# mfalxa/fakepta

Measured on AMD Instinct MI355X. Metric: residual samples/sec (TOA×realization) for 100-psr HD GWB; % FP64 peak, higher is better.
Workload: dtype f64

## Files before the change

fakepta_amd/csrc/fused_sched.h:

```cpp
#pragma once
#include <cstdint>

#if defined(__HIPCC__)
#define FPTA_SCHED_HD __host__ __device__
#else
#define FPTA_SCHED_HD
#endif

namespace fpta {

constexpr int kFusedShapeAny = 0;
constexpr int kFusedShapeGenLoad = 1;
constexpr int kFusedShapeLoad = 2;
constexpr int kFusedSlotAny = -1, kFusedSlotNone = 0, kFusedSlotGen = 1, kFusedSlotLoad = 2;
FPTA_SCHED_HD constexpr int fused_shape_nsig(int shape) {
  return shape == kFusedShapeGenLoad ? 2 : shape == kFusedShapeLoad ? 1 : 0;
}
FPTA_SCHED_HD constexpr int fused_shape_slot(int shape, int s, int i) {
  return shape == kFusedShapeAny       ? kFusedSlotAny
         : shape == kFusedShapeGenLoad ? (i == 0 ? kFusedSlotGen : (s == 0 && i == 1 ? kFusedSlotLoad : kFusedSlotNone))
                                       : (s == 0 && i == 0 ? kFusedSlotLoad : kFusedSlotNone);
}

FPTA_SCHED_HD constexpr int fused_shape_match(int n_sig, const int32_t* n_terms, const int32_t (*kind)[2]) {
  return n_sig == 2 && n_terms[0] == 2 && kind[0][0] == 0 && kind[0][1] == 1 && n_terms[1] == 1 && kind[1][0] == 0
             ? kFusedShapeGenLoad
         : n_sig == 1 && n_terms[0] == 1 && kind[0][0] == 1 ? kFusedShapeLoad
                                                            : kFusedShapeAny;
}

FPTA_SCHED_HD constexpr int32_t fused_ksteps(int32_t nm, int par) { return (((nm + (par ? 0 : 1)) >> 1) + 3) >> 2; }
FPTA_SCHED_HD constexpr int32_t fused_groups(int32_t nm) { return (fused_ksteps(nm, 0) + 1) >> 1; }

FPTA_SCHED_HD constexpr int32_t fused_iterations(int32_t ng0, int32_t ng1) { return ng0 > ng1 ? ng0 : ng1; }
FPTA_SCHED_HD constexpr bool fused_steps(int32_t jng, int32_t g) { return g < jng; }
FPTA_SCHED_HD constexpr bool fused_draw_loads(int32_t ng_s, int32_t g, bool last) { return last || g + 1 < ng_s; }
FPTA_SCHED_HD constexpr bool fused_draws(int32_t ng_s, int32_t g, bool last, bool nx) { return last ? nx : g + 1 < ng_s; }
FPTA_SCHED_HD constexpr int32_t fused_draw_group(int32_t g, bool last) { return last ? 0 : g + 1; }

}

#undef FPTA_SCHED_HD
```

fakepta_amd/csrc/grid_fused.hip:

```cpp
#include <hip/hip_runtime.h>
#include <hip/hip_ext.h>
#include <algorithm>
#include <atomic>
#include <type_traits>

#include "fused_device.h"

namespace fpta {

#ifndef FPTA_FUSED_DFT_PRIO
#define FPTA_FUSED_DFT_PRIO 3
#endif
#ifndef FPTA_HALF_STORE16
#define FPTA_HALF_STORE16 0
#endif
#ifndef FPTA_HALF_AHEAD
#define FPTA_HALF_AHEAD 2
#endif
constexpr int kFusedHalfAhead = FPTA_HALF_AHEAD;
#ifndef FPTA_HALF_PIN
#define FPTA_HALF_PIN 0
#endif

#ifndef FPTA_FUSED_CUT
#define FPTA_FUSED_CUT 0
#endif

namespace {

template <int NS>
struct FusedOps {
  int c;
  i32x4 ci;
  dbl2 b[NS];
  int row[NS];
};
template <int NS>
struct FusedOpsH {
  int c;
  i32x4 ci;
  dbl2 b[2][NS / 2];
  int row[2][NS];
};

__device__ __forceinline__ uint32_t dpp_u32_xor1(uint32_t x) {
  return (uint32_t)__builtin_amdgcn_update_dpp(0, (int)x, 0xB1, 0xF, 0xF, false);
}
__device__ __forceinline__ void bm_half(uint32_t wl, uint32_t wa, double& zc, double& zs) {
  double sn, cs;
  const double r = bm_sqrt(-2.0 * bm_log_u32(wl));
  bm_sincos2pi_u32(wa, sn, cs);
  zc = r * cs;
  zs = r * sn;
}
__device__ __forceinline__ void fused_mix_tile(const FusedMix& m, int k, int rg, int pg, int lane) {
  constexpr int NT = kFusedMixGroup / 16;
  const int lr = lane & 15, lg = lane >> 4;
  const int r = 16 * rg + lr;
  const bool rv = r < m.n_real;
  const uint64_t g = (uint64_t)(m.real0 + r);
  const int p0 = kFusedMixGroup * pg;
  int qe[NT];
  int qmax = 0;
#pragma unroll
  for (int t = 0; t < NT; ++t) {
    const int pt = p0 + 16 * t;
    qe[t] = pt < m.P ? min(m.lower ? min(m.P, pt + 16) : m.P, m.n_q) : 0;
    qmax = max(qmax, qe[t]);
  }
  d4 acc[NT][2];
#pragma unroll
  for (int t = 0; t < NT; ++t) acc[t][0] = acc[t][1] = d4{0.0, 0.0, 0.0, 0.0};
  const double* __restrict__ lt = m.LT + p0 + lr;
  const bool paired = (m.real0 & 1) == 0;
  const int e = lr & 1;
  const uint32_t ctr3 = (uint32_t)(g >> 1);
  for (int q0 = 0; q0 < qmax; q0 += 8) {
    double a0[NT], a1[NT];
#pragma unroll
    for (int t = 0; t < NT; ++t) {
      a0[t] = q0 < qe[t] ? ld_global(lt + (int64_t)(q0 + lg) * m.lt_ld + 16 * t) : 0.0;
      a1[t] = q0 + 4 < qe[t] ? ld_global(lt + (int64_t)(q0 + 4 + lg) * m.lt_ld + 16 * t) : 0.0;
    }
    double zc0, zs0, zc1, zs1;
    if (paired) {
      const u32x4 v = philox4x32_10({(uint32_t)k, (uint32_t)(q0 + 4 * e + lg), (uint32_t)m.seg, ctr3}, m.k0, m.k1);
      const uint32_t r0 = dpp_u32_xor1(e ? v.x : v.z), r1 = dpp_u32_xor1(e ? v.y : v.w);
      bm_half(e ? r0 : v.x, e ? r1 : v.y, zc0, zs0);
      bm_half(e ? v.z : r0, e ? v.w : r1, zc1, zs1);
    } else {
      gp_normal2((uint32_t)k, (uint32_t)(q0 + lg), (uint32_t)m.seg, g, m.k0, m.k1, zc0, zs0);
      gp_normal2((uint32_t)k, (uint32_t)(q0 + 4 + lg), (uint32_t)m.seg, g, m.k0, m.k1, zc1, zs1);
    }
    const bool ok0 = rv && q0 + lg < m.n_q, ok1 = rv && q0 + 4 + lg < m.n_q;
    zc0 = ok0 ? zc0 : 0.0;
    zs0 = ok0 ? zs0 : 0.0;
    zc1 = ok1 ? zc1 : 0.0;
    zs1 = ok1 ? zs1 : 0.0;
#pragma unroll
    for (int t = 0; t < NT; ++t)
      if (q0 < qe[t]) {
        acc[t][0] = __builtin_amdgcn_mfma_f64_16x16x4f64(a0[t], zc0, acc[t][0], 0, 0, 0);
        acc[t][1] = __builtin_amdgcn_mfma_f64_16x16x4f64(a0[t], zs0, acc[t][1], 0, 0, 0);
      }
#pragma unroll
    for (int t = 0; t < NT; ++t)
      if (q0 + 4 < qe[t]) {
        acc[t][0] = __builtin_amdgcn_mfma_f64_16x16x4f64(a1[t], zc1, acc[t][0], 0, 0, 0);
        acc[t][1] = __builtin_amdgcn_mfma_f64_16x16x4f64(a1[t], zs1, acc[t][1], 0, 0, 0);
      }
  }
  const double am = ld_global(m.amp + k);
#pragma unroll
  for (int t = 0; t < NT; ++t)
#pragma unroll
    for (int h = 0; h < 2; ++h)
#pragma unroll
      for (int gg = 0; gg < 4; ++gg) {
        const int p = p0 + 16 * t + lg + 4 * gg;
        if (p < m.P) m.coef[((int64_t)p * m.K + m.col0 + 2 * k + h) * m.R_pad + r] = am * acc[t][h][gg];
      }
}

}

template <int NQ, bool ODD, bool GEN, bool HALF, int SHAPE>
__device__ __forceinline__ void grid_fused_body(const SynthArgs& a, const GridBand& band, const FusedArgs& f,
                                                int32_t n_rb, int32_t n_items) {
  static_assert(kFusedTerms == 2 && kFusedMaxSig == 2, "fused_shape_slot's slots and signals (c0, c1)");
  static_assert(SHAPE == kFusedShapeAny || GEN == (SHAPE == kFusedShapeGenLoad), "a shape fixes whether terms are drawn");
  static_assert(kFusedReal == 32 && kFusedPitch == 32 && kFusedGroupModes * kFusedReal / 2 == 64 * kFusedDW,
                "two realization tiles; one (mode, realization pair) of a 16-mode group per DFT lane");
  static_assert(!HALF || (NQ % 4 == 0 && kGridTT == 2 * kFusedHalfTT), "half bands: whole row groups, two halves");
  extern __shared__ __attribute__((aligned(16))) double lds[];
  const FusedQueue queue(n_items, f.queue);
  const int wave = __builtin_amdgcn_readfirstlane(threadIdx.x >> 6);
  const int lane = threadIdx.x & 63;
  const int lr = lane & 15, lg = lane >> 4;
  double* __restrict__ ring = lds + f.ring_off;
  uint32_t* sync = (uint32_t*)(ring + 2 * kFusedMaxSig * kFusedSlot);
  volatile int* qitem = (volatile int*)(sync + 4);
  if (threadIdx.x == 0) {
    *sync = 0u;
    ((volatile int*)sync)[8] = 0;
    ((volatile int*)sync)[9] = 0;
    qitem[0] = queue.fetch();
    qitem[1] = qitem[0] >= 0 ? queue.fetch() : -1;
  }
  __syncthreads();
  auto item_of = [&](int k) { return __builtin_amdgcn_readfirstlane(qitem[k & 3]); };
  auto finish = [&]() {
    if (threadIdx.x == 0) {
      __threadfence();
      const uint32_t done = __hip_atomic_fetch_add(f.queue + 8, 1u, __ATOMIC_ACQ_REL, __HIP_MEMORY_SCOPE_AGENT);
      if (done == gridDim.x - 1)
        for (int i = 0; i < kFusedQueueWords; ++i)
          __hip_atomic_store(f.queue + i, 0u, __ATOMIC_RELAXED, __HIP_MEMORY_SCOPE_AGENT);
    }
  };
  auto mix_tiles = [&]() {
    if (f.mix.n_tiles <= 0) return;
    __builtin_amdgcn_s_setprio(0);
    const int n_pg = (f.mix.P + kFusedMixGroup - 1) / kFusedMixGroup, n_rg = f.mix.R_pad >> 4;
    for (;;) {
      int t = 0;
      if (lane == 0)
        t = (int)__hip_atomic_fetch_add(f.queue + kFusedMixWord, 1u, __ATOMIC_RELAXED, __HIP_MEMORY_SCOPE_AGENT);
      t = __builtin_amdgcn_readfirstlane(t);
      if (t >= f.mix.n_tiles) break;
      const int pg = t % n_pg, kr = t / n_pg;
      const int k = kr / n_rg;
      fused_mix_tile(f.mix, k, kr - k * n_rg, pg, lane);
    }
  };
  if (item_of(0) < 0) {
    finish();
    return;
  }

  volatile int* ccnt = (volatile int*)(sync + 8);
  struct Geo {
    int p, r0, c0, n;
    int64_t toa0;
    bool valid;
  };
  auto geo = [&](int k) {
    Geo g;
    const int item = item_of(k);
    g.valid = item >= 0;
    const int it = g.valid ? item : 0;
    g.p = it / n_rb;
    g.r0 = (it - g.p * n_rb) * kFusedReal;
    g.c0 = ld_uniform(f.psr_c0 + g.p);
    g.n = g.valid ? ld_uniform(f.psr_c0 + g.p + 1) - g.c0 : 0;
    g.toa0 = ld_uniform(a.offs + g.p);
    return g;
  };
  auto ticket = [&](int k) {
    int t = 0;
    if (lane == 0)
      t = __hip_atomic_fetch_add((int*)ccnt + (k & 1), 1, __ATOMIC_RELAXED, __HIP_MEMORY_SCOPE_WORKGROUP);
    return __builtin_amdgcn_readfirstlane(t);
  };
  auto lane_now = [&]() {
    int v = lane;
    asm volatile("" : "+v"(v));
    return v;
  };
  using Ops = typename std::conditional<HALF, FusedOpsH<NQ>, FusedOps<NQ>>::type;
  using OpsJ = typename std::conditional<HALF, FusedOpsH<NQ>, FusedOps<(NQ < 8 ? NQ : 8)>>::type;
  auto load_half = [&](int cc, auto& o, int ln) {
    {
      constexpr int NS = sizeof(o.row[0]) / sizeof(o.row[0][0]);
      o.c = cc;
      o.ci = *(const i32x4*)(f.h.chunks + cc);
      const int lgo = ln >> 4, lro = ln & 15;
#pragma unroll
      for (int h = 0; h < 2; ++h) {
        const i32x4* __restrict__ rt = (const i32x4*)(f.h.lrows + (((int64_t)cc * 2 + h) * 4 + lgo) * f.h.fq);
#pragma unroll
        for (int q4 = 0; q4 < NS / 4; ++q4) {
          const i32x4 r4 = rt[q4];
          o.row[h][4 * q4] = r4.x;
          o.row[h][4 * q4 + 1] = r4.y;
          o.row[h][4 * q4 + 2] = r4.z;
          o.row[h][4 * q4 + 3] = r4.w;
        }
        const double* __restrict__ wp =
            f.h.wd + ((int64_t)cc * 2 + h) * f.h.vmax * kFusedHalfTT + (lgo * kFusedHalfTT + lro) * 2;
#pragma unroll
        for (int qp = 0; qp < NS / 2; ++qp) o.b[h][qp] = *(const dbl2*)(wp + qp * 8 * kFusedHalfTT);
      }
    }
  };
  auto load_full = [&](int cc, auto& o, int ln) {
    constexpr int NS = sizeof(o.row) / sizeof(o.row[0]);
    o.c = cc;
    o.ci = *(const i32x4*)(band.chunks + cc);
    const int lgo = ln >> 4, lro = ln & 15;
    const i32x4* __restrict__ rt = (const i32x4*)(f.lrows + ((int64_t)cc * 4 + lgo) * f.fq);
    const double* __restrict__ wp = band.wd + ((int64_t)cc * band.vmax + lgo) * kGridTT + 2 * lro;
#pragma unroll
    for (int q4 = 0; q4 < NS / 4; ++q4) {
      const i32x4 r4 = rt[q4];
      o.row[4 * q4] = r4.x;
      o.row[4 * q4 + 1] = r4.y;
      o.row[4 * q4 + 2] = r4.z;
      o.row[4 * q4 + 3] = r4.w;
    }
#pragma unroll
    for (int q = 0; q < NS; ++q) o.b[q] = *(const dbl2*)(wp + 4 * kGridTT * q);
  };
  auto load = [&](int cc, auto& o, int ln) {
    if constexpr (HALF)
      load_half(cc, o, ln);
    else
      load_full(cc, o, ln);
  };
  auto process_half = [&](const Geo& g, const auto& cur, auto& pf, int ln) {
    constexpr int NS = sizeof(cur.row[0]) / sizeof(cur.row[0][0]);
    const int lg = ln >> 4, lr = ln & 15;
    const int lds_lane = 2 * lr;
    const int ty = __builtin_amdgcn_readfirstlane(cur.ci.y), tc = __builtin_amdgcn_readfirstlane(cur.ci.z);
    const int nqw = __builtin_amdgcn_readfirstlane(cur.ci.w);
    const int nq[2] = {nqw & 0xFFFF, nqw >> 16};
    FPTA_DCHECK(nq[0] > 0, "k_grid_fused half band steps", nq[0], 1 << 20);
    d4 acc[2][2];
#pragma unroll
    for (int h = 0; h < 2; ++h)
#pragma unroll
      for (int i = 0; i < 2; ++i) acc[h][i] = d4{0.0, 0.0, 0.0, 0.0};
    {
      constexpr int DA = kFusedHalfAhead;
      const int nqm = min(max(nq[0], nq[1]), NS);
      dbl2 an[2][NS];
      auto rd = [&](int q) {
#pragma unroll
        for (int h = 0; h < 2; ++h) an[h][q] = *(const dbl2*)(lds + cur.row[h][q] * kFusedPitch + lds_lane);
      };
#pragma unroll
      for (int q = 0; q < DA && q < NS; ++q) rd(q);
#pragma unroll
      for (int q = 0; q < NS; ++q) {
        if (q < nqm) {
          if (q + DA < NS) rd(q + DA);
          if (FPTA_HALF_PIN) __builtin_amdgcn_sched_barrier(0);
          const double b0 = (q & 1) ? cur.b[0][q >> 1].y : cur.b[0][q >> 1].x;
          const double b1 = (q & 1) ? cur.b[1][q >> 1].y : cur.b[1][q >> 1].x;
          acc[0][0] = __builtin_amdgcn_mfma_f64_16x16x4f64(an[0][q].x, b0, acc[0][0], 0, 0, 0);
          acc[0][1] = __builtin_amdgcn_mfma_f64_16x16x4f64(an[0][q].y, b0, acc[0][1], 0, 0, 0);
          acc[1][0] = __builtin_amdgcn_mfma_f64_16x16x4f64(an[1][q].x, b1, acc[1][0], 0, 0, 0);
          acc[1][1] = __builtin_amdgcn_mfma_f64_16x16x4f64(an[1][q].y, b1, acc[1][1], 0, 0, 0);
        }
      }
    }
    pf.lap(1);
#pragma unroll
    for (int h = 0; h < 2; ++h)
      for (int q = NS; q < nq[h]; ++q) {
        const int64_t hc = (int64_t)cur.c * 2 + h;
        const int row = f.h.lrows[(hc * 4 + lg) * f.h.fq + q];
        const double bv = f.h.wd[hc * f.h.vmax * kFusedHalfTT + fused_half_weight_index(4 * q + lg, lr)];
        const dbl2 av = *(const dbl2*)(lds + row * kFusedPitch + lds_lane);
        acc[h][0] = __builtin_amdgcn_mfma_f64_16x16x4f64(av.x, bv, acc[h][0], 0, 0, 0);
        acc[h][1] = __builtin_amdgcn_mfma_f64_16x16x4f64(av.y, bv, acc[h][1], 0, 0, 0);
      }
    pf.lap(4);
    __builtin_amdgcn_sched_barrier(0);
    const int64_t t0 = g.toa0 + ty;
    if ((FPTA_FUSED_CUT & 8) && acc[0][0][0] != -1.25e300) return;
    if (FPTA_HALF_STORE16 && tc == kGridTT && g.r0 + kFusedReal <= a.n_real && ((t0 | a.ldo) & 1) == 0 &&
        a.ldo < ((int64_t)1 << 26)) {
      const bool odd = lr & 1;
      const uint32_t vo = (uint32_t)(((int64_t)2 * lg * a.ldo + (odd ? 15 + lr : lr)) * 8);
      const char* base = (const char*)(a.out + t0 + (int64_t)g.r0 * a.ldo);
#pragma unroll
      for (int i = 0; i < 2; ++i)
#pragma unroll
        for (int gg = 0; gg < 4; ++gg) {
          const double send = odd ? acc[0][i][gg] : acc[1][i][gg];
          const double recv = dpp_xor1(send);
          const dbl2 v = odd ? dbl2{recv, acc[1][i][gg]} : dbl2{acc[0][i][gg], recv};
          __builtin_nontemporal_store(v, (dbl2*)((char*)base + (int64_t)(8 * gg + i) * a.ldo * 8 + vo));
        }
    } else if (tc == kGridTT && g.r0 + kFusedReal <= a.n_real && a.ldo < ((int64_t)1 << 26)) {
      const uint32_t vo = (uint32_t)(((int64_t)2 * lg * a.ldo + lr) * 8);
      const char* base = (const char*)(a.out + t0 + (int64_t)g.r0 * a.ldo);
#pragma unroll
      for (int h = 0; h < 2; ++h)
#pragma unroll
        for (int i = 0; i < 2; ++i)
#pragma unroll
          for (int gg = 0; gg < 4; ++gg)
            __builtin_nontemporal_store(acc[h][i][gg],
                                        (double*)((char*)base + ((int64_t)(8 * gg + i) * a.ldo + 16 * h) * 8 + vo));
    } else {
#pragma unroll
      for (int h = 0; h < 2; ++h) {
        if (16 * h + lr >= tc) continue;
#pragma unroll
        for (int i = 0; i < 2; ++i)
#pragma unroll
          for (int gg = 0; gg < 4; ++gg) {
            const int r = g.r0 + 2 * (lg + 4 * gg) + i;
            if (r < a.n_real) a.out[t0 + 16 * h + lr + (int64_t)r * a.ldo] = acc[h][i][gg];
          }
      }
    }
    pf.lap(2);
  };
  auto process_full = [&](const Geo& g, const auto& cur, auto& pf, int ln) {
    constexpr int NS = sizeof(cur.row) / sizeof(cur.row[0]);
    const int lg = ln >> 4, lr = ln & 15;
    const int lds_lane = 2 * lr;
    const int ty = __builtin_amdgcn_readfirstlane(cur.ci.y), tc = __builtin_amdgcn_readfirstlane(cur.ci.z);
    const int nq = __builtin_amdgcn_readfirstlane(cur.ci.w) >> 2;
    FPTA_DCHECK(nq > 0, "k_grid_fused band steps", nq, 1 << 20);
    d4 acc[2][2];
#pragma unroll
    for (int e = 0; e < 2; ++e)
#pragma unroll
      for (int i = 0; i < 2; ++i) acc[e][i] = d4{0.0, 0.0, 0.0, 0.0};
    {
      dbl2 an = *(const dbl2*)(lds + cur.row[0] * kFusedPitch + lds_lane);
#pragma unroll
      for (int q = 0; q < NS; ++q) {
        if (q < nq) {
          const dbl2 av = an;
          if (q + 1 < NS) an = *(const dbl2*)(lds + cur.row[q + 1] * kFusedPitch + lds_lane);
          const dbl2 bv = cur.b[q];
          acc[0][0] = __builtin_amdgcn_mfma_f64_16x16x4f64(av.x, bv.x, acc[0][0], 0, 0, 0);
          acc[0][1] = __builtin_amdgcn_mfma_f64_16x16x4f64(av.y, bv.x, acc[0][1], 0, 0, 0);
          acc[1][0] = __builtin_amdgcn_mfma_f64_16x16x4f64(av.x, bv.y, acc[1][0], 0, 0, 0);
          acc[1][1] = __builtin_amdgcn_mfma_f64_16x16x4f64(av.y, bv.y, acc[1][1], 0, 0, 0);
        }
      }
    }
    pf.lap(1);
    for (int q = NS; q < nq; ++q) {
      const int v = 4 * q + lg;
      const int row = f.lrows[((int64_t)cur.c * 4 + lg) * f.fq + q];
      const dbl2 bv = *(const dbl2*)(band.wd + ((int64_t)cur.c * band.vmax + v) * kGridTT + 2 * lr);
      const dbl2 av = *(const dbl2*)(lds + row * kFusedPitch + lds_lane);
      acc[0][0] = __builtin_amdgcn_mfma_f64_16x16x4f64(av.x, bv.x, acc[0][0], 0, 0, 0);
      acc[0][1] = __builtin_amdgcn_mfma_f64_16x16x4f64(av.y, bv.x, acc[0][1], 0, 0, 0);
      acc[1][0] = __builtin_amdgcn_mfma_f64_16x16x4f64(av.x, bv.y, acc[1][0], 0, 0, 0);
      acc[1][1] = __builtin_amdgcn_mfma_f64_16x16x4f64(av.y, bv.y, acc[1][1], 0, 0, 0);
    }
    pf.lap(4);
    __builtin_amdgcn_sched_barrier(0);
    const int64_t t0 = g.toa0 + ty;
    if ((FPTA_FUSED_CUT & 8) && acc[0][0][0] != -1.25e300) return;
    if (FPTA_HALF_STORE16 && tc == kGridTT && g.r0 + kFusedReal <= a.n_real && ((t0 | a.ldo) & 1) == 0 &&
        a.ldo < ((int64_t)1 << 26)) {
      const uint32_t vo = (uint32_t)(((int64_t)2 * lg * a.ldo + 2 * lr) * 8);
      const char* base = (const char*)(a.out + t0 + (int64_t)g.r0 * a.ldo);
#pragma unroll
      for (int i = 0; i < 2; ++i)
#pragma unroll
        for (int gg = 0; gg < 4; ++gg)
          __builtin_nontemporal_store(dbl2{acc[0][i][gg], acc[1][i][gg]},
                                      (dbl2*)((char*)base + (int64_t)(8 * gg + i) * a.ldo * 8 + vo));
    } else {
      InterpTile<2> t;
      t.c = cur.c;
      t.p = g.p;
      t.r0 = g.r0;
      t.y = ty;
      t.cnt = tc;
      t.nq = nq;
      interp_store_rows<2>(a, a.out, t, acc);
    }
    pf.lap(2);
  };
  auto process = [&](const Geo& g, const auto& cur, auto& pf, int ln) {
    if constexpr (HALF)
      process_half(g, cur, pf, ln);
    else
      process_full(g, cur, pf, ln);
  };

  if (wave >= kFusedIW) {
    const int dw = wave - kFusedIW;
    __builtin_amdgcn_s_setprio(FPTA_FUSED_DFT_PRIO);
    constexpr int kNSig = fused_shape_nsig(SHAPE);
    const int n_sig = kNSig ? kNSig : f.n_sig;
    int js = -1, jrc = 0;
    {
      int j = dw;
#pragma unroll
      for (int s = 0; s < kFusedMaxSig; ++s) {
        if (s < n_sig && js < 0 && j < f.s[s].n_rc) {
          js = s;
          jrc = j;
        }
        if (s < n_sig) j -= f.s[s].n_rc;
      }
    }
    js = __builtin_amdgcn_readfirstlane(js);
    jrc = __builtin_amdgcn_readfirstlane(jrc);
    Prof pf;
    pf.start();
    uint32_t epoch = 0;
    auto dsync = [&]() {
      fused_wait_lgkm0();
      if (lane == 0) __hip_atomic_fetch_add(sync, 1u, __ATOMIC_RELAXED, __HIP_MEMORY_SCOPE_WORKGROUP);
      epoch += kFusedDW;
      while ((uint32_t)__builtin_amdgcn_readfirstlane(
                 (int)__hip_atomic_load(sync, __ATOMIC_RELAXED, __HIP_MEMORY_SCOPE_WORKGROUP)) < epoch)
        __builtin_amdgcn_s_sleep(1);
    };
    int ng[kFusedMaxSig];
#pragma unroll
    for (int s = 0; s < kFusedMaxSig; ++s) ng[s] = s < n_sig ? fused_groups(f.s[s].nm) : 0;
    const int n_it = fused_iterations(ng[0], ng[1]);
    const FusedSig& jf = f.s[js < 0 ? 0 : js];
    const int64_t jts = (int64_t)jf.ntq * jf.ldq, jld4 = 4 * (int64_t)jf.ldq;
    auto jtq_now = [&]() {
      const int ln = lane_now();
      return jf.tq + (int64_t)(ln >> 4) * jf.ldq + 32 * jrc + 2 * (ln & 15);
    };
    const int jnq0 = fused_ksteps(jf.nm, 0), jnq1 = fused_ksteps(jf.nm, 1);
    const int jng = js < 0 ? 0 : fused_groups(jf.nm);
    d4 C[2][2][2], S[2][2][2];
    struct DrawIn {
      dbl2 x0[kFusedTerms], x1[kFusedTerms];
    };
    std::integral_constant<int, 0> c0;
    std::integral_constant<int, 1> c1;
    auto draw_load = [&](auto sc, int g, int p, int r0, DrawIn& in) {
      constexpr int s = decltype(sc)::value;
      const FusedSig& fs = f.s[s];
      const int didx = dw * 64 + lane_now(), dmm = didx >> 4, drl = 2 * (didx & 15);
      const int m = kFusedGroupModes * g + dmm, r = r0 + drl;
      auto slot = [&](auto ic) {
        constexpr int i = decltype(ic)::value, kind = fused_shape_slot(SHAPE, s, i);
        if constexpr (kind == kFusedSlotGen) {
          const int nmi = fs.term_nm[i], mi = min(m, nmi - 1);
          in.x0[i] = ld_global((const dbl2*)(fs.term_amp[i] + (int64_t)p * nmi + (mi & ~1)));
        } else if constexpr (kind == kFusedSlotLoad) {
          const int mi = min(m, fs.term_nm[i] - 1);
          const double* src0 = a.coef + ((int64_t)p * a.K + fs.term_col0[i] + 2 * mi) * a.R_pad + r;
          in.x0[i] = ld_global((const dbl2*)src0);
          in.x1[i] = ld_global((const dbl2*)(src0 + a.R_pad));
        } else if constexpr (kind == kFusedSlotAny) {
          const bool on = i < fs.n_terms;
          const int nmi = on ? fs.term_nm[i] : 2;
          const int mi = min(m, nmi - 1);
          const double* src0;
          int64_t step;
          if (on && fs.term_kind[i] == 1) {
            src0 = a.coef + ((int64_t)p * a.K + fs.term_col0[i] + 2 * mi) * a.R_pad + r;
            step = a.R_pad;
          } else {
            src0 = (on ? fs.term_amp[i] : a.coef) + (int64_t)p * nmi + (mi & ~1);
            step = 0;
          }
          in.x0[i] = ld_global((const dbl2*)src0);
          in.x1[i] = ld_global((const dbl2*)(src0 + step));
        }
      };
      slot(c0);
      slot(c1);
    };
    auto draw_finish = [&](auto sc, int g, int p, int r0, double* __restrict__ slot_s, const DrawIn& in) {
      constexpr int s = decltype(sc)::value;
      const FusedSig& fs = f.s[s];
      const int didx = dw * 64 + lane_now(), dmm = didx >> 4, drl = 2 * (didx & 15);
      const int m = kFusedGroupModes * g + dmm, r = r0 + drl;
      const uint64_t gr = (uint64_t)(f.real0 + r);
      double bc[2] = {0.0, 0.0}, bs[2] = {0.0, 0.0};
      bool first = true;
      auto add = [&](bool use, const double (&pc)[2], const double (&ps)[2]) {
#pragma unroll
        for (int h = 0; h < 2; ++h) {
          bc[h] = use ? (first ? pc[h] : bc[h] + pc[h]) : bc[h];
          bs[h] = use ? (first ? ps[h] : bs[h] + ps[h]) : bs[h];
        }
        first = first && !use;
      };
      const bool ok0 = r < a.n_real, ok1 = r + 1 < a.n_real;
      auto normals = [&](int seg, double (&z)[4]) {
        uint32_t k0 = f.k0, k1 = f.k1;
        if (SHAPE != kFusedShapeAny) asm volatile("" : "+s"(k0), "+s"(k1));
        if (!ODD) {
          gp_pair2((uint32_t)m, (uint32_t)p, (uint32_t)seg, gr, k0, k1, z);
        } else {
          gp_normal2((uint32_t)m, (uint32_t)p, (uint32_t)seg, gr, k0, k1, z[0], z[1]);
          gp_normal2((uint32_t)m, (uint32_t)p, (uint32_t)seg, gr + 1, k0, k1, z[2], z[3]);
        }
        z[0] = ok0 ? z[0] : 0.0;
        z[1] = ok0 ? z[1] : 0.0;
        z[2] = ok1 ? z[2] : 0.0;
        z[3] = ok1 ? z[3] : 0.0;
      };
      auto term = [&](auto ic) {
        constexpr int i = decltype(ic)::value, kind = fused_shape_slot(SHAPE, s, i);
        if (kind == kFusedSlotNone || (kind == kFusedSlotAny && i >= fs.n_terms)) return;
        double pc[2], ps[2];
        if (kind == kFusedSlotGen || (kind == kFusedSlotAny && GEN && fs.term_kind[i] == 0)) {
          double z[4];
          normals(fs.term_seg[i], z);
          const double amp = (m & 1) ? in.x0[i].y : in.x0[i].x;
          pc[0] = opaque(amp * z[0]);
          ps[0] = opaque(amp * z[1]);
          pc[1] = opaque(amp * z[2]);
          ps[1] = opaque(amp * z[3]);
        } else {
          pc[0] = in.x0[i].x;
          pc[1] = in.x0[i].y;
          ps[0] = in.x1[i].x;
          ps[1] = in.x1[i].y;
        }
        add(m < fs.nm && m < fs.term_nm[i], pc, ps);
      };
      term(c0);
      term(c1);
      for (int i = kFusedTerms; SHAPE == kFusedShapeAny && i < fs.n_terms; ++i) {
        const int mi = min(m, fs.term_nm[i] - 1);
        double pc[2], ps[2];
        if (GEN && fs.term_kind[i] == 0) {
          double z[4];
          normals(fs.term_seg[i], z);
          const double amp = ld_global(fs.term_amp[i] + (int64_t)p * fs.term_nm[i] + mi);
          pc[0] = opaque(amp * z[0]);
          ps[0] = opaque(amp * z[1]);
          pc[1] = opaque(amp * z[2]);
          ps[1] = opaque(amp * z[3]);
        } else {
          const double* cp = a.coef + ((int64_t)p * a.K + fs.term_col0[i] + 2 * mi) * a.R_pad + r;
          const dbl2 vc = ld_global((const dbl2*)cp), vs = ld_global((const dbl2*)(cp + a.R_pad));
          pc[0] = vc.x;
          pc[1] = vc.y;
          ps[0] = vs.x;
          ps[1] = vs.y;
        }
        add(m < fs.nm && m < fs.term_nm[i], pc, ps);
      }
      double* __restrict__ dst = slot_s + 2 * (dmm * kFusedReal + drl);
      *(dbl2*)dst = dbl2{bc[0], bs[0]};
      *(dbl2*)(dst + 2) = dbl2{bc[1], bs[1]};
    };
    auto slot_of = [&](int k, int s) { return ring + ((k & 1) * kFusedMaxSig + s) * kFusedSlot; };
    struct Tabs {
      dbl2 ac[2][2], as[2][2];
    };
    auto tables = [&](int g, Tabs& tb) {
#pragma unroll
      for (int h2 = 0; h2 < 2; ++h2) {
        const int q = max(0, min(2 * g + h2, jnq0 - 1));
#pragma unroll
        for (int par = 0; par < 2; ++par) {
          const double* __restrict__ tc = jtq_now() + (int64_t)(2 * par) * jts + q * jld4;
          tb.ac[h2][par] = ld_global((const dbl2*)tc);
          tb.as[h2][par] = ld_global((const dbl2*)(tc + jts));
        }
      }
    };
    auto steps = [&](int slot, int g, const Tabs& tb) {
      const double* __restrict__ bsrc = slot_of(slot, js);
#pragma unroll
      for (int h2 = 0; h2 < 2; ++h2) {
        const int q = 2 * g + h2;
#pragma unroll
        for (int par = 0; par < 2; ++par) {
          if (q >= (par ? jnq1 : jnq0)) continue;
          const dbl2 ac = tb.ac[h2][par], as = tb.as[h2][par];
          const double* bm = bsrc + 2 * ((2 * (4 * h2 + lg) + par) * kFusedReal + lr);
          const dbl2 b[2] = {*(const dbl2*)bm, *(const dbl2*)(bm + 2 * 16)};
#pragma unroll
          for (int t = 0; t < 2; ++t) {
            C[par][0][t] = __builtin_amdgcn_mfma_f64_16x16x4f64(ac.x, b[t].x, C[par][0][t], 0, 0, 0);
            C[par][1][t] = __builtin_amdgcn_mfma_f64_16x16x4f64(ac.y, b[t].x, C[par][1][t], 0, 0, 0);
            S[par][0][t] = __builtin_amdgcn_mfma_f64_16x16x4f64(as.x, b[t].y, S[par][0][t], 0, 0, 0);
            S[par][1][t] = __builtin_amdgcn_mfma_f64_16x16x4f64(as.y, b[t].y, S[par][1][t], 0, 0, 0);
          }
        }
      }
    };
    int sb = 0;
    auto build = [&](int k) {
      const int item = item_of(k);
      const int p = item / n_rb, r0 = (item - p * n_rb) * kFusedReal;
      const int item1n = item_of(k + 1);
      const bool nx = item1n >= 0;
      const int item1 = nx ? item1n : item;
      const int p1 = item1 / n_rb, r1 = (item1 - p1 * n_rb) * kFusedReal;
#pragma unroll
      for (int par = 0; par < 2; ++par)
#pragma unroll
        for (int h = 0; h < 2; ++h)
#pragma unroll
          for (int t = 0; t < 2; ++t) C[par][h][t] = S[par][h][t] = d4{0.0, 0.0, 0.0, 0.0};
      if (k == 0) {
        auto first = [&](auto sc) {
          constexpr int s = decltype(sc)::value;
          if (s >= n_sig) return;
          DrawIn in;
          draw_load(sc, 0, p, r0, in);
          draw_finish(sc, 0, p, r0, slot_of(sb, s), in);
        };
        first(c0);
        first(c1);
        pf.lap(6);
        dsync();
        pf.lap(2);
      }
      constexpr bool kAny = SHAPE == kFusedShapeAny;
      for (int g = 0; g < n_it; ++g) {
        const bool last = g + 1 == n_it;
        const int dp = last ? p1 : p, dr = last ? r1 : r0;
        Tabs tb;
        if (kAny) tables(g, tb);
        DrawIn in[kFusedMaxSig];
        auto load = [&](auto sc) {
          constexpr int s = decltype(sc)::value;
          if (kAny || (s < kNSig && fused_draw_loads(ng[s], g, last)))
            draw_load(sc, last ? 0 : min(g + 1, max(ng[s], 1) - 1), dp, dr, in[s]);
        };
        load(c0);
        load(c1);
        if (!kAny && fused_steps(jng, g)) tables(g, tb);
        pf.lap(0);
        if (fused_steps(jng, g)) steps(sb + g, g, tb);
        pf.lap(1);
        auto finish_draw = [&](auto sc) {
          constexpr int s = decltype(sc)::value;
          if (s < n_sig && fused_draws(ng[s], g, last, nx))
            draw_finish(sc, fused_draw_group(g, last), dp, dr, slot_of(sb + g + 1, s), in[s]);
        };
        finish_draw(c0);
        finish_draw(c1);
        pf.lap(6);
        if (!kAny) fused_wait_vm0();
        dsync();
        pf.lap(2);
        pf.count(5);
      }
      sb = (sb + n_it) & 1;
    };
    auto write_grid = [&]() {
      if (js >= 0) {
        const int j0 = 32 * jrc;
        const int nf = jf.nf, Q = nf >> 2, H = nf >> 1;
        double* __restrict__ gcol = lds + (int64_t)jf.lrow0 * kFusedPitch + lr;
#pragma unroll
        for (int h = 0; h < 2; ++h)
#pragma unroll
          for (int gg = 0; gg < 4; ++gg) {
            const int j = j0 + 2 * (lg + 4 * gg) + h;
            if (j > Q) continue;
#pragma unroll
            for (int t = 0; t < 2; ++t) {
              const double oc = C[0][h][t][gg], os = S[0][h][t][gg], ec = C[1][h][t][gg], es = S[1][h][t][gg];
              const double pe = ec + es, me = ec - es, po = oc + os, mo = oc - os;
              gcol[j * kFusedPitch + 16 * t] = pe + po;
              gcol[(H + j) * kFusedPitch + 16 * t] = pe - po;
              if (j > 0 && j < Q) {
                gcol[(H - j) * kFusedPitch + 16 * t] = me - mo;
                gcol[(nf - j) * kFusedPitch + 16 * t] = me + mo;
              }
            }
          }
      }
      fused_wait_lgkm0();
    };
    auto join = [&](int k) {
      if (FPTA_FUSED_CUT & 6) return;
      const Geo g = geo(k);
      auto take = [&]() {
        if (__builtin_amdgcn_readfirstlane(ccnt[k & 1]) >= g.n - f.join_reserve) return -1;
        const int t = ticket(k);
        return t < g.n ? t : -1;
      };
      int t = take();
      if (t < 0) return;
      OpsJ o0, o1;
      load(g.c0 + t, o0, lane_now());
      for (;;) {
        t = take();
        load(t >= 0 ? g.c0 + t : o0.c, o1, lane_now());
        process(g, o0, pf, lane_now());
        pf.count(7);
        if (t < 0) return;
        t = take();
        load(t >= 0 ? g.c0 + t : o1.c, o0, lane_now());
        process(g, o1, pf, lane_now());
        pf.count(7);
        if (t < 0) return;
      }
    };
    auto barrier_a = [&](int k) {
      fused_barrier();
      pf.lap(4);
      if (dw == 0 && lane == 0) ccnt[k & 1] = 0;
    };
    for (int k = -1;; ++k) {
      const bool next = item_of(k + 1) >= 0;
      if (dw == 0 && lane == 0) qitem[(k + 3) & 3] = item_of(k + 2) >= 0 ? queue.fetch() : -1;
      if (k >= 0) join(k);
      if (!next) break;
      if (!(FPTA_FUSED_CUT & 1)) build(k + 1);
      if (k >= 0) barrier_a(k);
      write_grid();
      pf.lap(3);
      fused_barrier();
      pf.lap(4);
    }
    pf.flush(f.prof, wave);
  } else {
  Prof pf;
  pf.start();
  fused_barrier();
  pf.lap(3);
  int k = 0;
  Geo g0 = geo(0), g1 = geo(1);
  bool ex0 = false, ex1 = false;
  auto next = [&](int& kn) {
    if (!ex0) {
      const int t = ticket(k);
      if (t < g0.n) {
        kn = k;
        return g0.c0 + t;
      }
      ex0 = true;
    }
    if (!ex1 && g1.valid) {
      const int t = ticket(k + 1);
      if (t < g1.n) {
        kn = k + 1;
        return g1.c0 + t;
      }
      ex1 = true;
    }
    kn = -1;
    return -1;
  };
  auto step = [&](Ops& cur, Ops& nxt, int& kc) {
    pf.lap(6);
    int kn;
    const int cn = next(kn);
    load(cn >= 0 ? cn : cur.c, nxt, lane);
    pf.lap(0);
    pf.count(5);
    if (!(FPTA_FUSED_CUT & 2)) process(g0, cur, pf, lane);
    kc = kn;
  };
  Ops o0, o1;
  int kc;
  {
    const int cc = next(kc);
    load(cc >= 0 ? cc : g0.c0, o0, lane);
  }
  for (;;) {
    while (kc == k) {
      step(o0, o1, kc);
      if (kc != k) {
        o0 = o1;
        break;
      }
      step(o1, o0, kc);
    }
    if (!g1.valid) break;
    fused_wait_lgkm0();
    pf.lap(6);
    fused_barrier();
    fused_barrier();
    pf.lap(3);
    ++k;
    g0 = g1;
    g1 = geo(k + 1);
    ex0 = ex1;
    ex1 = false;
    if (kc < 0) {
      const int cc = next(kc);
      load(cc >= 0 ? cc : g0.c0, o0, lane);
    }
  }
  pf.flush(f.prof, wave);
  }
  mix_tiles();
  fused_barrier();
  if (wave < kFusedIW) finish();
}

template <int NQ, bool ODD, bool GEN, bool HALF>
__global__ __launch_bounds__(64 * (kFusedIW + kFusedDW), 1) void k_grid_fused(SynthArgs a, GridBand band, FusedArgs f,
                                                                             int32_t n_rb, int32_t n_items) {
  grid_fused_body<NQ, ODD, GEN, HALF, GEN ? kFusedShapeGenLoad : kFusedShapeLoad>(a, band, f, n_rb, n_items);
}
template <int NQ, bool ODD, bool GEN, bool HALF>
__global__ __launch_bounds__(64 * (kFusedIW + kFusedDW), 1) void k_grid_fused_any(SynthArgs a, GridBand band,
                                                                                 FusedArgs f, int32_t n_rb,
                                                                                 int32_t n_items) {
  grid_fused_body<NQ, ODD, GEN, HALF, kFusedShapeAny>(a, band, f, n_rb, n_items);
}

#ifndef FPTA_FUSED_SHAPES
#define FPTA_FUSED_SHAPES 1
#endif
static int fused_shape_of(const FusedArgs& f) {
  int32_t n_terms[kFusedMaxSig], kind[kFusedMaxSig][2];
  for (int s = 0; s < kFusedMaxSig; ++s) {
    n_terms[s] = f.s[s].n_terms;
    kind[s][0] = f.s[s].term_kind[0];
    kind[s][1] = f.s[s].term_kind[1];
  }
  return FPTA_FUSED_SHAPES ? fused_shape_match(f.n_sig, n_terms, kind) : kFusedShapeAny;
}

hipError_t launch_grid_fused(hipStream_t st, const SynthArgs& a, const GridBand& band, const FusedArgs& f,
                             int32_t nq_max, size_t lds_bytes, hipEvent_t ev0, hipEvent_t ev1, bool half,
                             int* kernel_out, int* shape_out) {
  if (band.n_chunks <= 0 || band.vmax < 4 || f.join_reserve < 0 || band.vmax % 4 != 0 || a.R_pad % kFusedReal != 0 || a.w_on ||
      a.accumulate || a.part || !f.lrows || !f.psr_c0 || f.n_sig <= 0 || f.n_sig > kFusedMaxSig ||
      lds_bytes > (size_t)kFusedLdsMax || nq_max <= 0 || f.ring_off < 0 || f.fq < kFusedNQ || f.fq % 4 != 0 ||
      !f.queue || (size_t)(f.ring_off + 2 * kFusedMaxSig * kFusedSlot) * sizeof(double) + 48 > lds_bytes)
    return hipErrorInvalidValue;
  if (half && (!f.h.chunks || !f.h.lrows || !f.h.wd || f.h.fq < kFusedHalfNQ || f.h.fq % 4 != 0 || f.h.vmax < 8 ||
               f.h.vmax % 8 != 0))
    return hipErrorInvalidValue;
  int jobs = 0;
  for (int s = 0; s < f.n_sig; ++s) {
    const FusedSig& fs = f.s[s];
    const int nq = fused_ksteps(fs.nm, 0);
    if (fs.nf % 4 != 0 || !fs.tq || fs.n_rc != (fs.nf / 4 + 32) / 32 || fs.ldq < 32 * fs.n_rc || 4 * nq > fs.ntq ||
        fs.n_terms <= 0 || fs.n_terms > kDftGenTerms || fs.lrow0 < 0 || (fs.lrow0 + fs.nf) * kFusedPitch > f.ring_off)
      return hipErrorInvalidValue;
    for (int i = 0; i < fs.n_terms; ++i)
      if (fs.term_nm[i] <= 0 || fs.term_nm[i] > fs.nm || (fs.term_kind[i] == 0 && (!fs.term_amp[i] || fs.term_nm[i] % 2)) ||
          (fs.term_kind[i] == 1 && (!a.coef || fs.term_col0[i] < 0 || fs.term_col0[i] + 2 * fs.term_nm[i] > a.K)))
        return hipErrorInvalidValue;
    jobs += fs.n_rc;
  }
  if (jobs > kFusedDW) return hipErrorInvalidValue;
  const FusedMix& m = f.mix;
  if (m.n_tiles != 0 &&
      (m.n_tiles < 0 || !m.LT || !m.amp || !m.coef || m.P <= 0 || m.P > kFusedMixMaxP || m.lt_ld < 16 * ((m.P + 15) / 16) ||
       m.lt_rows < 4 * ((m.P + 3) / 4) || m.n_q <= 0 || m.n_q > m.P || m.nm <= 0 || m.R_pad <= 0 ||
       m.R_pad % 16 != 0 || m.n_real <= 0 || m.n_real > m.R_pad || (int64_t)m.n_tiles != (int64_t)m.nm * (m.R_pad / 16) * ((m.P + kFusedMixGroup - 1) / kFusedMixGroup) ||
       m.col0 < 0 || m.col0 + 2 * m.nm > m.K || m.real0 < 0 || m.real0 + m.n_real > ((int64_t)1 << 32)))
    return hipErrorInvalidValue;
  const int32_t n_rb = a.R_pad / kFusedReal;
  const int64_t items = (int64_t)a.P * n_rb;
  if (items > 0x7FFFFFFF || items <= 0) return hipErrorInvalidValue;
  int dev = 0;
  if (hipGetDevice(&dev) != hipSuccess || dev < 0 || dev >= 64) return hipErrorInvalidDevice;
  static std::atomic<int> n_cus[64];
  static std::atomic<bool> attr_set[64][2][kFusedKernels];
  int n_cu = n_cus[dev].load(std::memory_order_relaxed);
  if (n_cu <= 0) {
    if (hipDeviceGetAttribute(&n_cu, hipDeviceAttributeMultiprocessorCount, dev) != hipSuccess || n_cu <= 0) n_cu = 256;
    n_cus[dev].store(n_cu, std::memory_order_relaxed);
  }
  const int64_t cus = f.cu_pct > 0 && f.cu_pct < 100 ? std::max<int64_t>(8, (int64_t)n_cu * f.cu_pct / 100) : n_cu;
  const int64_t grid = std::min<int64_t>((items + 7) / 8 * 8, (cus + 7) / 8 * 8);
  bool gen = false;
  for (int s = 0; s < f.n_sig; ++s)
    for (int i = 0; i < f.s[s].n_terms; ++i) gen = gen || f.s[s].term_kind[i] == 0;
  const bool odd = gen && (f.real0 & 1);
  const int ki = half ? 6 + (gen ? 1 + odd : 0) : (nq_max <= 8 ? 0 : 3) + (gen ? 1 + odd : 0);
  using K = void (*)(SynthArgs, GridBand, FusedArgs, int32_t, int32_t);
  static const K kernels[2][kFusedKernels] = {
      {k_grid_fused_any<8, false, false, false>, k_grid_fused_any<8, false, true, false>,
       k_grid_fused_any<8, true, true, false>, k_grid_fused_any<12, false, false, false>,
       k_grid_fused_any<12, false, true, false>, k_grid_fused_any<12, true, true, false>,
       k_grid_fused_any<kFusedHalfNQ, false, false, true>, k_grid_fused_any<kFusedHalfNQ, false, true, true>,
       k_grid_fused_any<kFusedHalfNQ, true, true, true>},
      {k_grid_fused<8, false, false, false>, k_grid_fused<8, false, true, false>, k_grid_fused<8, true, true, false>,
       k_grid_fused<12, false, false, false>, k_grid_fused<12, false, true, false>, k_grid_fused<12, true, true, false>,
       k_grid_fused<kFusedHalfNQ, false, false, true>, k_grid_fused<kFusedHalfNQ, false, true, true>,
       k_grid_fused<kFusedHalfNQ, true, true, true>}};
  const int shaped = fused_shape_of(f) == (gen ? kFusedShapeGenLoad : kFusedShapeLoad) ? 1 : 0;
  const K kernel = kernels[shaped][ki];
  if (!attr_set[dev][shaped][ki].load(std::memory_order_acquire)) {
    hipError_t e = hipFuncSetAttribute((const void*)kernel, hipFuncAttributeMaxDynamicSharedMemorySize, kFusedLdsMax);
    if (e != hipSuccess) return e;
    attr_set[dev][shaped][ki].store(true, std::memory_order_release);
  }
  FusedArgs fa = f;
  for (int s = f.n_sig; s < kFusedMaxSig; ++s) fa.s[s] = f.s[0];
  (void)hipGetLastError();
  int32_t n_rb_arg = n_rb, items_arg = (int32_t)items;
  void* args[] = {(void*)&a, (void*)&band, (void*)&fa, (void*)&n_rb_arg, (void*)&items_arg};
  const hipError_t e = hipExtLaunchKernel((const void*)kernel, dim3((unsigned)grid),
                                          dim3(64 * (kFusedIW + kFusedDW)), args, lds_bytes, st, ev0, ev1, 0);
  if (e == hipSuccess && kernel_out) *kernel_out = ki;
  if (e == hipSuccess && shape_out) *shape_out = shaped ? (gen ? kFusedShapeGenLoad : kFusedShapeLoad) : kFusedShapeAny;
  return e;
}

}
```

Before: 392.7 billion.

## Add solo-draw scheduling to spread signal draws into idle iterations

Adds an opt-in schedule, off by default, for signals whose draws finish early. When a signal has one row chunk and two groups, a single owner wave draws the next item's group-1 quarters during the spare iterations, and the other waves skip their group-0 draw. The goal is to rebalance draw work across the pipeline. It also adds an always-on early return in draw_finish that skips generated-noise terms for quarters past the mode count, saving RNG work on dead lanes. The extra control flow and added register use could reduce occupancy.

```diff
diff --git a/fakepta_amd/csrc/fused_sched.h b/fakepta_amd/csrc/fused_sched.h
--- a/fakepta_amd/csrc/fused_sched.h
+++ b/fakepta_amd/csrc/fused_sched.h
@@ -38,6 +38,31 @@
 FPTA_SCHED_HD constexpr bool fused_draws(int32_t ng_s, int32_t g, bool last, bool nx) { return last ? nx : g + 1 < ng_s; }
 FPTA_SCHED_HD constexpr int32_t fused_draw_group(int32_t g, bool last) { return last ? 0 : g + 1; }
 
+FPTA_SCHED_HD constexpr bool fused_draw_live(int32_t nm, int32_t g, int32_t dw) { return 16 * g + 4 * dw < nm; }
+
+constexpr int32_t kFusedSoloQuarters = 3;
+FPTA_SCHED_HD constexpr bool fused_solo(int32_t n_rc_s, int32_t ng_s, int32_t n_it) {
+  return n_rc_s == 1 && ng_s == 2 && n_it - ng_s >= kFusedSoloQuarters;
+}
+FPTA_SCHED_HD constexpr int32_t fused_solo_owner(int s, int32_t n_rc0) { return s == 0 ? 0 : n_rc0; }
+FPTA_SCHED_HD constexpr int32_t fused_solo_quarter(int32_t ng_s, int32_t g, int32_t owner) {
+  return g >= ng_s && g < ng_s + kFusedSoloQuarters ? ((owner + 1 + g - ng_s) & 3) : -1;
+}
+FPTA_SCHED_HD constexpr bool fused_solo_draws(bool solo, int32_t ng_s, int32_t g, int32_t dw, int32_t owner, bool nx) {
+  return solo && nx && dw == owner && fused_solo_quarter(ng_s, g, owner) >= 0;
+}
+FPTA_SCHED_HD constexpr bool fused_solo_skips(bool solo, int32_t g, bool last, int32_t dw, int32_t owner, bool first) {
+  return solo && !last && g == 0 && !first && dw != owner;
+}
+FPTA_SCHED_HD constexpr bool fused_draw_loads_solo(bool solo, int32_t ng_s, int32_t g, bool last, int32_t dw,
+                                                   int32_t owner, bool first) {
+  return fused_draw_loads(ng_s, g, last) && !fused_solo_skips(solo, g, last, dw, owner, first);
+}
+FPTA_SCHED_HD constexpr bool fused_draws_solo(bool solo, int32_t ng_s, int32_t g, bool last, bool nx, int32_t dw,
+                                              int32_t owner, bool first) {
+  return fused_draws(ng_s, g, last, nx) && !fused_solo_skips(solo, g, last, dw, owner, first);
+}
+
 }
 
 #undef FPTA_SCHED_HD
diff --git a/fakepta_amd/csrc/grid_fused.hip b/fakepta_amd/csrc/grid_fused.hip
--- a/fakepta_amd/csrc/grid_fused.hip
+++ b/fakepta_amd/csrc/grid_fused.hip
@@ -10,6 +10,9 @@
 
 #ifndef FPTA_FUSED_DFT_PRIO
 #define FPTA_FUSED_DFT_PRIO 3
+#endif
+#ifndef FPTA_FUSED_SOLO_DRAWS
+#define FPTA_FUSED_SOLO_DRAWS 0
 #endif
 #ifndef FPTA_HALF_STORE16
 #define FPTA_HALF_STORE16 0
@@ -454,6 +457,7 @@
 #pragma unroll
     for (int s = 0; s < kFusedMaxSig; ++s) ng[s] = s < n_sig ? fused_groups(f.s[s].nm) : 0;
     const int n_it = fused_iterations(ng[0], ng[1]);
+    constexpr bool kSolo = FPTA_FUSED_SOLO_DRAWS && SHAPE != kFusedShapeAny && kNSig > 1;
     const FusedSig& jf = f.s[js < 0 ? 0 : js];
     const int64_t jts = (int64_t)jf.ntq * jf.ldq, jld4 = 4 * (int64_t)jf.ldq;
     auto jtq_now = [&]() {
@@ -468,10 +472,10 @@
     };
     std::integral_constant<int, 0> c0;
     std::integral_constant<int, 1> c1;
-    auto draw_load = [&](auto sc, int g, int p, int r0, DrawIn& in) {
+    auto draw_load = [&](auto sc, int g, int qw, int p, int r0, DrawIn& in) {
       constexpr int s = decltype(sc)::value;
       const FusedSig& fs = f.s[s];
-      const int didx = dw * 64 + lane_now(), dmm = didx >> 4, drl = 2 * (didx & 15);
+      const int didx = qw * 64 + lane_now(), dmm = didx >> 4, drl = 2 * (didx & 15);
       const int m = kFusedGroupModes * g + dmm, r = r0 + drl;
       auto slot = [&](auto ic) {
         constexpr int i = decltype(ic)::value, kind = fused_shape_slot(SHAPE, s, i);
@@ -503,10 +507,10 @@
       slot(c0);
       slot(c1);
     };
-    auto draw_finish = [&](auto sc, int g, int p, int r0, double* __restrict__ slot_s, const DrawIn& in) {
+    auto draw_finish = [&](auto sc, int g, int qw, int p, int r0, double* __restrict__ slot_s, const DrawIn& in) {
       constexpr int s = decltype(sc)::value;
       const FusedSig& fs = f.s[s];
-      const int didx = dw * 64 + lane_now(), dmm = didx >> 4, drl = 2 * (didx & 15);
+      const int didx = qw * 64 + lane_now(), dmm = didx >> 4, drl = 2 * (didx & 15);
       const int m = kFusedGroupModes * g + dmm, r = r0 + drl;
       const uint64_t gr = (uint64_t)(f.real0 + r);
       double bc[2] = {0.0, 0.0}, bs[2] = {0.0, 0.0};
@@ -537,6 +541,7 @@
       auto term = [&](auto ic) {
         constexpr int i = decltype(ic)::value, kind = fused_shape_slot(SHAPE, s, i);
         if (kind == kFusedSlotNone || (kind == kFusedSlotAny && i >= fs.n_terms)) return;
+        if (kind == kFusedSlotGen && !fused_draw_live(min(fs.nm, fs.term_nm[i]), g, qw)) return;
         double pc[2], ps[2];
         if (kind == kFusedSlotGen || (kind == kFusedSlotAny && GEN && fs.term_kind[i] == 0)) {
           double z[4];
@@ -637,8 +642,8 @@
           constexpr int s = decltype(sc)::value;
           if (s >= n_sig) return;
           DrawIn in;
-          draw_load(sc, 0, p, r0, in);
-          draw_finish(sc, 0, p, r0, slot_of(sb, s), in);
+          draw_load(sc, 0, dw, p, r0, in);
+          draw_finish(sc, 0, dw, p, r0, slot_of(sb, s), in);
         };
         first(c0);
         first(c1);
@@ -647,16 +652,33 @@
         pf.lap(2);
       }
       constexpr bool kAny = SHAPE == kFusedShapeAny;
+      bool solo[kFusedMaxSig];
+      int owner[kFusedMaxSig];
+#pragma unroll
+      for (int s = 0; s < kFusedMaxSig; ++s) {
+        solo[s] = kSolo && s < n_sig && fused_solo(f.s[s].n_rc, ng[s], n_it);
+        owner[s] = fused_solo_owner(s, f.s[0].n_rc);
+      }
       for (int g = 0; g < n_it; ++g) {
         const bool last = g + 1 == n_it;
         const int dp = last ? p1 : p, dr = last ? r1 : r0;
         Tabs tb;
         if (kAny) tables(g, tb);
         DrawIn in[kFusedMaxSig];
+        int qs[kFusedMaxSig];
+        bool reg_ld[kFusedMaxSig];
+#pragma unroll
+        for (int s = 0; s < kFusedMaxSig; ++s) {
+          qs[s] = kSolo && fused_solo_draws(solo[s], ng[s], g, dw, owner[s], nx) ? fused_solo_quarter(ng[s], g, owner[s]) : -1;
+          reg_ld[s] = kSolo ? fused_draw_loads_solo(solo[s], ng[s], g, last, dw, owner[s], k == 0)
+                            : fused_draw_loads(ng[s], g, last);
+        }
         auto load = [&](auto sc) {
           constexpr int s = decltype(sc)::value;
-          if (kAny || (s < kNSig && fused_draw_loads(ng[s], g, last)))
-            draw_load(sc, last ? 0 : min(g + 1, max(ng[s], 1) - 1), dp, dr, in[s]);
+          if (kAny || (s < kNSig && reg_ld[s]))
+            draw_load(sc, last ? 0 : min(g + 1, max(ng[s], 1) - 1), dw, dp, dr, in[s]);
+          else if (kSolo && s < kNSig && qs[s] >= 0)
+            draw_load(sc, 1, qs[s], p1, r1, in[s]);
         };
         load(c0);
         load(c1);
@@ -666,8 +688,18 @@
         pf.lap(1);
         auto finish_draw = [&](auto sc) {
           constexpr int s = decltype(sc)::value;
-          if (s < n_sig && fused_draws(ng[s], g, last, nx))
-            draw_finish(sc, fused_draw_group(g, last), dp, dr, slot_of(sb + g + 1, s), in[s]);
+          if (s >= n_sig) return;
+          if (!kSolo) {
+            if (fused_draws(ng[s], g, last, nx))
+              draw_finish(sc, fused_draw_group(g, last), dw, dp, dr, slot_of(sb + g + 1, s), in[s]);
+            return;
+          }
+          const bool reg = fused_draws_solo(solo[s], ng[s], g, last, nx, dw, owner[s], k == 0);
+          for (int ps = reg ? 0 : 1; ps < (qs[s] >= 0 ? 2 : 1); ++ps) {
+            if (ps && reg_ld[s]) draw_load(sc, 1, qs[s], p1, r1, in[s]);
+            draw_finish(sc, ps ? 1 : fused_draw_group(g, last), ps ? qs[s] : dw, ps ? p1 : dp, ps ? r1 : dr,
+                        slot_of(ps ? sb + n_it + 1 : sb + g + 1, s), in[s]);
+          }
         };
         finish_draw(c0);
         finish_draw(c1);
```

Result: no change. 395.9 billion (median of 6 runs) (+0.8%).
